# anonymousauthors001/SGS-GNN

Hardware: AMD Instinct MI355X
Metric: sampled edges/sec + training steps/sec, Reddit hybrid 20% sparsity (higher is better)
Workload: dtype f32

## Files before the change

### sgs-gnn_amd/csrc/gemm_tn.hip

```cpp
#include "sgs_common.h"

namespace sgs {
namespace {

using f32x16 = __attribute__((ext_vector_type(16))) float;
constexpr int kUnroll = 8;

__global__ void __launch_bounds__(64) gemm_tn_tile(const float* __restrict__ A, const float* __restrict__ B, int64_t K, int M, int N,
                                                  int ksplit, float* __restrict__ slab) {
    const int lane = threadIdx.x, kh = lane >> 5, l31 = lane & 31;
    const int ti = blockIdx.x, tj = blockIdx.y, s = blockIdx.z;
    const int i = ti * 32 + l31, j = tj * 32 + l31;
    const bool iok = i < M, jok = j < N;
    const int64_t per = ((K + ksplit - 1) / ksplit + 1) & ~int64_t(1);
    const int64_t k0 = s * per, k1 = (k0 + per < K) ? k0 + per : K;
    f32x16 acc;
#pragma unroll
    for (int r = 0; r < 16; ++r) acc[r] = 0.f;
    int64_t k = k0;
    for (; k + 2 * kUnroll <= k1; k += 2 * kUnroll) {
        float a[kUnroll], b[kUnroll];
#pragma unroll
        for (int u = 0; u < kUnroll; ++u) {
            const int64_t kk = k + 2 * u + kh;
// ... 376 lines not shown
                Bp[w][0][m] = p1; Bp[w][1][m] = p2; Bp[w][2][m] = p3;
            }
        if constexpr (MASK) {
#pragma unroll
            for (int t = 0; t < 4; ++t) {
                u32x4 A1;
#pragma unroll
                for (int m = 0; m < 4; ++m)
                    A1[m] = ((r.aw[2 * m] >> t) & 1u) * 0x3F80u + ((r.aw[2 * m + 1] >> t) & 1u) * 0x3F800000u;
                const bf16x8 a1 = __builtin_bit_cast(bf16x8, A1);
#pragma unroll
                for (int w = 0; w < 2; ++w) {
                    if constexpr (ONE) {
                        acc[t][w] = __builtin_amdgcn_mfma_f32_32x32x16_bf16(a1, __builtin_bit_cast(bf16x8, Bp[w][0]), acc[t][w], 0, 0, 0);
                        continue;
                    }
                    const bf16x8 b1 = __builtin_bit_cast(bf16x8, Bp[w][0]), b2 = __builtin_bit_cast(bf16x8, Bp[w][1]), b3 = __builtin_bit_cast(bf16x8, Bp[w][2]);
                    acc[t][w] = __builtin_amdgcn_mfma_f32_32x32x16_bf16(a1, b3, acc[t][w], 0, 0, 0);
                    acc[t][w] = __builtin_amdgcn_mfma_f32_32x32x16_bf16(a1, b2, acc[t][w], 0, 0, 0);
                    acc[t][w] = __builtin_amdgcn_mfma_f32_32x32x16_bf16(a1, b1, acc[t][w], 0, 0, 0);
                }
            }
            return;
        }
#pragma unroll
        for (int t = 0; t < 4; ++t) {
            u32x4 Ap[3];
#pragma unroll
            for (int m = 0; m < 4; ++m) {
                const float4 lo = r.a[2 * m], hi = r.a[2 * m + 1];
                const float e0 = t == 0 ? lo.x : t == 1 ? lo.y : t == 2 ? lo.z : lo.w;
                const float e1 = t == 0 ? hi.x : t == 1 ? hi.y : t == 2 ? hi.z : hi.w;
                uint32_t p1, p2, p3;
                split3(e0, e1, p1, p2, p3);
                Ap[0][m] = p1; Ap[1][m] = p2; Ap[2][m] = p3;
            }
            const bf16x8 a1 = __builtin_bit_cast(bf16x8, Ap[0]), a2 = __builtin_bit_cast(bf16x8, Ap[1]), a3 = __builtin_bit_cast(bf16x8, Ap[2]);
#pragma unroll
            for (int w = 0; w < 2; ++w) {
                const bf16x8 b1 = __builtin_bit_cast(bf16x8, Bp[w][0]), b2 = __builtin_bit_cast(bf16x8, Bp[w][1]), b3 = __builtin_bit_cast(bf16x8, Bp[w][2]);
                acc[t][w] = __builtin_amdgcn_mfma_f32_32x32x16_bf16(a3, b1, acc[t][w], 0, 0, 0);
                acc[t][w] = __builtin_amdgcn_mfma_f32_32x32x16_bf16(a2, b2, acc[t][w], 0, 0, 0);
                acc[t][w] = __builtin_amdgcn_mfma_f32_32x32x16_bf16(a1, b3, acc[t][w], 0, 0, 0);
                acc[t][w] = __builtin_amdgcn_mfma_f32_32x32x16_bf16(a2, b1, acc[t][w], 0, 0, 0);
                acc[t][w] = __builtin_amdgcn_mfma_f32_32x32x16_bf16(a1, b2, acc[t][w], 0, 0, 0);
                acc[t][w] = __builtin_amdgcn_mfma_f32_32x32x16_bf16(a1, b1, acc[t][w], 0, 0, 0);
            }
        }
    };
    Raw r0, r1;
    if constexpr (GATHER) {
        if (lim > 0) {
            Raw r2;
            Idx ix;
            load_idx(k0, ix);
            load_rows(k0, r0, ix);
            load_idx(k0 + 16, ix);
            load_rows(k0 + 16, r1, ix);
            load_idx(k0 + 32, ix);
#pragma unroll 1
            for (int64_t k = k0; k < k1; k += 48) {
                load_rows(k + 32, r2, ix);
                load_idx(k + 48, ix);
                mma(r0);
                load_rows(k + 48, r0, ix);
                load_idx(k + 64, ix);
                mma(r1);
                load_rows(k + 64, r1, ix);
                load_idx(k + 80, ix);
                mma(r2);
            }
        }
    } else if constexpr (!MASK) {
        load(k0, r0);
    } else {
        if (lim > 0) load(k0, r0);
    }
    if constexpr (MASK && !GATHER) {
        if (lim > 0) {
        Raw r2;
        load(k0 + 16, r1);
#pragma unroll 1
        for (int64_t k = k0; k < k1; k += 48) {
            load(k + 32, r2);
            mma(r0);
            load(k + 48, r0);
            mma(r1);
            load(k + 64, r1);
            mma(r2);
        }
        }
    } else if constexpr (!MASK) {
#pragma unroll 1
        for (int64_t k = k0; k < k1; k += 32) {
            load(k + 16, r1);
            mma(r0);
            load(k + 32, r0);
            mma(r1);
        }
    }
    if (want_cs) {
#pragma unroll
        for (int t = 0; t < 4; ++t) cs[t] += __shfl_xor(cs[t], 32, 64);
    }
    if (want_dz) {
        dzs += __shfl_xor(dzs, 32, 64);
        if (lane == 0) dzpart[s] = dzs;
    }
    if (NW > 1) {
        float* csl = red_lds + (NW / 2) * 128 * 64;
#pragma unroll
        for (int half = NW / 2; half >= 1; half >>= 1) {
            if (wave >= half && wave < 2 * half) {
                float* dstp = red_lds + static_cast<size_t>(wave - half) * 128 * 64;
#pragma unroll
                for (int t = 0; t < 4; ++t)
#pragma unroll
                    for (int u = 0; u < 2; ++u)
#pragma unroll
                        for (int r = 0; r < 16; ++r) dstp[((t * 2 + u) * 16 + r) * 64 + lane] = acc[t][u][r];
#pragma unroll
                for (int t = 0; t < 4; ++t) csl[((wave - half) * 4 + t) * 64 + lane] = cs[t];
            }
            __syncthreads();
            if (wave < half) {
                const float* srcp = red_lds + static_cast<size_t>(wave) * 128 * 64;
#pragma unroll
                for (int t = 0; t < 4; ++t)
#pragma unroll
                    for (int u = 0; u < 2; ++u)
#pragma unroll
                        for (int r = 0; r < 16; ++r) acc[t][u][r] += srcp[((t * 2 + u) * 16 + r) * 64 + lane];
#pragma unroll
                for (int t = 0; t < 4; ++t) cs[t] += csl[(wave * 4 + t) * 64 + lane];
            }
            __syncthreads();
        }
        if (wave != 0) return;
    }
    const int slab_id = blockIdx.z;
    if (want_cs && g == 0 && aok) *reinterpret_cast<float4*>(cpart + static_cast<int64_t>(slab_id) * M + ia) = make_float4(cs[0], cs[1], cs[2], cs[3]);
    float* out = slab + static_cast<int64_t>(slab_id) * M * N;
    if (bok) {
#pragma unroll
        for (int t = 0; t < 4; ++t)
#pragma unroll
            for (int r = 0; r < 16; ++r) {
                const int row = m0 + 4 * ((r & 3) + 8 * (r >> 2) + 4 * g) + t;
                if (row < M) *reinterpret_cast<float2*>(out + static_cast<int64_t>(row) * N + jb) = make_float2(acc[t][0][r], acc[t][1][r]);
            }
    }
}

constexpr int maskfeat_stage_words(int MT, int P) { return 2 * P * 64 * 4 + (128 * MT / 32) * 16 + 16; }
constexpr int maskfeat_lds_words(int MT, int P) {
    return 2 * 3 * maskfeat_stage_words(MT, P) > 4 * 2 * 16 * 64 + 4 * MT * 64 + 8 ? 2 * 3 * maskfeat_stage_words(MT, P) : 4 * 2 * 16 * 64 + 4 * MT * 64 + 8;
}
template <int MT, int NG, int P = 3>
__global__ void __launch_bounds__(512) gemm_tn_maskfeat(const uint32_t* __restrict__ Abits, const float* __restrict__ dz,
                                                        const float* __restrict__ codes, const int2* __restrict__ sd, int64_t K, int N,
                                                        float* __restrict__ slab, float* __restrict__ cpart, float* __restrict__ dzpart) {
    constexpr int M = 128 * MT, WPR = M / 32;
    constexpr int kBst = 2 * P * 64 * 4;
    constexpr int kMst = WPR * 16;
    constexpr int kStage = kBst + kMst + 16;
    extern __shared__ uint32_t lds[];
    const int lane = threadIdx.x & 63, g = lane >> 5, l31 = lane & 31;
    const int wave = __builtin_amdgcn_readfirstlane(threadIdx.x >> 6);
    const int kg = wave >> 2, w = wave & 3;
    const int ng = blockIdx.x, n0 = ng * 64, slab_id = blockIdx.y;
    const int64_t per = (((K + gridDim.y - 1) / gridDim.y) + 63) & ~int64_t(63);
    const int64_t kb = static_cast<int64_t>(slab_id) * per + kg * (per >> 1);
    const int64_t ke = (kb + (per >> 1) < K) ? kb + (per >> 1) : K;
    const int nsteps = static_cast<int>(per >> 5);
    const int lim = static_cast<int>(ke - kb);
    uint32_t* st0 = lds + kg * (3 * kStage);
    f32x16 acc[MT][2];
#pragma unroll
    for (int t = 0; t < MT; ++t)
#pragma unroll
        for (int u = 0; u < 2; ++u)
#pragma unroll
            for (int r = 0; r < 16; ++r) acc[t][u][r] = 0.f;
    float cs[MT];
#pragma unroll
    for (int t = 0; t < MT; ++t) cs[t] = 0.f;
    float dzs = 0.f;
    const bool want_cs = cpart != nullptr, want_dz = dzpart != nullptr && ng == 0;
    constexpr int rpg = 8 / NG;
    const int tid_g = threadIdx.x & 255;
    const int srow = (tid_g / WPR) & 15, sword = tid_g % WPR;
    const bool stage_mask = tid_g < 16 * WPR, stage_dz = w == 3 && lane < 16;
    struct S1 { int2 ea, eb; float da, db; uint32_t mw; float dl; };
    struct S2 { float2 as, ad, bs, bd; float da, db; uint32_t mw; float dl; };
    const int64_t kbase = lim > 0 ? kb : 0;
    const int2* sdb = sd + kbase;
    const float* dzb = dz + kbase;
    const uint32_t* abb = Abits + kbase * WPR;
    const int last = lim > 0 ? lim - 1 : 0;
    auto clampr = [&](int rel) { return static_cast<uint32_t>(max(min(rel, last), 0)); };
    const uint32_t coff = static_cast<uint32_t>(n0 + 2 * l31);
    auto load_idx = [&](int step) {
        S1 o;
        const int rel = 16 * step + 8 * g + 2 * w;
        const uint32_t ra = clampr(rel), rb = clampr(rel + 1);
        o.ea = sdb[ra]; o.eb = sdb[rb];
        o.da = dzb[ra]; o.db = dzb[rb];
        o.mw = abb[clampr(16 * step + srow) * WPR + sword];
        o.dl = dzb[clampr(16 * step + (lane & 15))];
        return o;
    };
    auto load_rows = [&](const S1& i) {
        S2 o;
        const uint32_t un = static_cast<uint32_t>(N);
        o.as = *reinterpret_cast<const float2*>(codes + (static_cast<uint32_t>(i.ea.x) * un + coff));
        o.ad = *reinterpret_cast<const float2*>(codes + (static_cast<uint32_t>(i.ea.y) * un + coff));
        o.bs = *reinterpret_cast<const float2*>(codes + (static_cast<uint32_t>(i.eb.x) * un + coff));
        o.bd = *reinterpret_cast<const float2*>(codes + (static_cast<uint32_t>(i.eb.y) * un + coff));
        o.da = i.da; o.db = i.db; o.mw = i.mw; o.dl = i.dl;
        return o;
    };
    auto publish = [&](const S2& r, int step, uint32_t* stg) {
        const int rel = 16 * step + 8 * g + 2 * w;
        const float da = rel < lim ? r.da : 0.f, db = rel + 1 < lim ? r.db : 0.f;
        const float a0 = (r.as.x * r.ad.x) * da, a1 = (r.as.y * r.ad.y) * da;
        const float b0 = (r.bs.x * r.bd.x) * db, b1 = (r.bs.y * r.bd.y) * db;
        if constexpr (P == 1) {
            stg[((0 * P + 0) * 64 + lane) * 4 + w] = pk_bf16(a0, b0);
            stg[((1 * P + 0) * 64 + lane) * 4 + w] = pk_bf16(a1, b1);
        } else {
        uint32_t p1, p2, p3;
        split3(a0, b0, p1, p2, p3);
        stg[((0 * 3 + 0) * 64 + lane) * 4 + w] = p1; stg[((0 * 3 + 1) * 64 + lane) * 4 + w] = p2; stg[((0 * 3 + 2) * 64 + lane) * 4 + w] = p3;
        split3(a1, b1, p1, p2, p3);
        stg[((1 * 3 + 0) * 64 + lane) * 4 + w] = p1; stg[((1 * 3 + 1) * 64 + lane) * 4 + w] = p2; stg[((1 * 3 + 2) * 64 + lane) * 4 + w] = p3;
        }
        if (stage_mask) stg[kBst + sword * 16 + srow] = r.mw;
        if (stage_dz) stg[kBst + kMst + lane] = __float_as_uint(16 * step + lane < lim ? r.dl : 0.f);
        if (want_dz && l31 == 0) dzs += da + db;
    };
    const int wsel = MT * w + ((MT * l31) >> 5), wsh = (MT * l31) & 31;
    struct Ops { bf16x8 bq[2][3]; uint4 m0, m1; uint32_t cw[8 / NG]; float cd[8 / NG]; };
    auto fetch = [&](const uint32_t* stg, Ops& o) {
        o.m0 = *reinterpret_cast<const uint4*>(stg + kBst + wsel * 16 + 8 * g);
        o.m1 = *reinterpret_cast<const uint4*>(stg + kBst + wsel * 16 + 8 * g + 4);
#pragma unroll
        for (int u = 0; u < 2; ++u)
#pragma unroll
            for (int pc = 0; pc < P; ++pc)
                o.bq[u][pc] = __builtin_bit_cast(bf16x8, *reinterpret_cast<const uint4*>(stg + ((u * P + pc) * 64 + lane) * 4));
        if (want_cs) {
#pragma unroll
            for (int jj = 0; jj < rpg; ++jj) {
                const int j = 8 * g + ng * rpg + jj;
                o.cw[jj] = stg[kBst + wsel * 16 + j];
                o.cd[jj] = __uint_as_float(stg[kBst + kMst + j]);
            }
        }
    };
    auto mma = [&](const Ops& o) {
        uint32_t aw[8] = {o.m0.x, o.m0.y, o.m0.z, o.m0.w, o.m1.x, o.m1.y, o.m1.z, o.m1.w};
#pragma unroll
        for (int j = 0; j < 8; ++j) aw[j] >>= wsh;
        uint32_t c[4];
#pragma unroll
        for (int m = 0; m < 4; ++m) c[m] = (aw[2 * m] & ((1u << MT) - 1u)) | ((aw[2 * m + 1] & ((1u << MT) - 1u)) << 16);
#pragma unroll
        for (int t = 0; t < MT; ++t) {
            u32x4 A1;
#pragma unroll
            for (int m = 0; m < 4; ++m) A1[m] = __umul24((c[m] >> t) & 0x00010001u, 0x3F80u);
            const bf16x8 a1 = __builtin_bit_cast(bf16x8, A1);
#pragma unroll
            for (int u = 0; u < 2; ++u) {
                if constexpr (P == 1) {
                    acc[t][u] = __builtin_amdgcn_mfma_f32_32x32x16_bf16(a1, o.bq[u][0], acc[t][u], 0, 0, 0);
                    continue;
                }
                acc[t][u] = __builtin_amdgcn_mfma_f32_32x32x16_bf16(a1, o.bq[u][2], acc[t][u], 0, 0, 0);
                acc[t][u] = __builtin_amdgcn_mfma_f32_32x32x16_bf16(a1, o.bq[u][1], acc[t][u], 0, 0, 0);
                acc[t][u] = __builtin_amdgcn_mfma_f32_32x32x16_bf16(a1, o.bq[u][0], acc[t][u], 0, 0, 0);
            }
        }
        if (want_cs) {
#pragma unroll
            for (int jj = 0; jj < rpg; ++jj) {
                const uint32_t wv = o.cw[jj] >> wsh;
#pragma unroll
                for (int t = 0; t < MT; ++t) cs[t] += (wv >> t) & 1u ? o.cd[jj] : 0.f;
            }
        }
    };
    {
        S1 ia = load_idx(0);
        S2 ra = load_rows(ia);
        S1 ib = load_idx(1);
        S2 rb = load_rows(ib);
        ia = load_idx(2);
        publish(ra, 0, st0);
        int sa = 0, sb = 1;
        if (kg == 1) __syncthreads();
        Ops op;
#pragma unroll 1
        for (int i = 0; i < nsteps; i += 2) {
            ra = load_rows(ia);
            ib = load_idx(i + 3);
            publish(rb, i + 1, st0 + sb * kStage);
            __syncthreads();
            fetch(st0 + sa * kStage, op);
            mma(op);
            __syncthreads();
            sa = sb; sb = sb == 2 ? 0 : sb + 1;
            rb = load_rows(ib);
            ia = load_idx(i + 4);
            publish(ra, i + 2, st0 + sb * kStage);
            __syncthreads();
            fetch(st0 + sa * kStage, op);
            mma(op);
            __syncthreads();
            sa = sb; sb = sb == 2 ? 0 : sb + 1;
        }
        if (kg == 0) __syncthreads();
    }
    if (want_cs) {
#pragma unroll
        for (int t = 0; t < MT; ++t) cs[t] += __shfl_xor(cs[t], 32, 64);
    }
    dzs += __shfl_xor(dzs, 32, 64);
    float* red = reinterpret_cast<float*>(lds);
    constexpr int kRedCs = 4 * 2 * 16 * 64, kRedDz = kRedCs + 4 * MT * 64;
    static_assert(kRedDz + 8 <= maskfeat_lds_words(MT, P) && 2 * 3 * kStage <= maskfeat_lds_words(MT, P), "the K-group sum reuses the stages");
#pragma unroll
    for (int t = 0; t < MT; ++t) {
        __syncthreads();
        if (t == 0 && lane == 0) red[kRedDz + wave] = dzs;
        if (kg == 1) {
#pragma unroll
            for (int u = 0; u < 2; ++u)
#pragma unroll
                for (int r = 0; r < 16; ++r) red[((w * 2 + u) * 16 + r) * 64 + lane] = acc[t][u][r];
            if (t == 0) {
#pragma unroll
                for (int tt = 0; tt < MT; ++tt) red[kRedCs + (w * MT + tt) * 64 + lane] = cs[tt];
            }
        }
        __syncthreads();
        if (kg == 0) {
#pragma unroll
            for (int u = 0; u < 2; ++u)
#pragma unroll
                for (int r = 0; r < 16; ++r) acc[t][u][r] += red[((w * 2 + u) * 16 + r) * 64 + lane];
            if (t == 0) {
#pragma unroll
                for (int tt = 0; tt < MT; ++tt) cs[tt] += red[kRedCs + (w * MT + tt) * 64 + lane];
                if (want_dz && wave == 0 && lane == 0) {
                    float a = 0.f;
                    for (int z = 0; z < 8; ++z) a += red[kRedDz + z];
                    dzpart[slab_id] = a;
                }
            }
        }
    }
    if (kg != 0) return;
    float* out = slab + static_cast<int64_t>(slab_id) * M * N;
#pragma unroll
    for (int t = 0; t < MT; ++t)
#pragma unroll
        for (int r = 0; r < 16; ++r) {
            const int h = 32 * MT * w + MT * ((r & 3) + 8 * (r >> 2) + 4 * g) + t;
            *reinterpret_cast<float2*>(out + static_cast<int64_t>(h) * N + n0 + 2 * l31) = make_float2(acc[t][0][r], acc[t][1][r]);
        }
    if (want_cs && g == 0) {
        float* cp = cpart + (static_cast<int64_t>(slab_id) * NG + ng) * M + 32 * MT * w + MT * l31;
#pragma unroll
        for (int t = 0; t < MT; ++t) cp[t] = cs[t];
    }
}

constexpr int kMaskfeatMaxSlabs = 128;
inline bool use_tall(int64_t K, int64_t M, int64_t N) { return K >= kTallK && M % 4 == 0 && N % 2 == 0; }
inline int pick_ksplit_tall(int64_t K, int64_t M, int64_t N) {
    const int64_t tiles = cdiv(M, 128) * cdiv(N, 64);
    int ks = 1;
    while (ks < 512 && tiles * ks < 1024 && K / (ks * 2) >= 256) ks *= 2;
    return ks;
}

inline int pick_ksplit(int64_t K, int64_t M, int64_t N) {
    if (use_tall(K, M, N)) return pick_ksplit_tall(K, M, N);
    const int64_t tiles = cdiv(M, 32) * cdiv(N, 32);
    int ks = 1;
    while (ks < 64 && tiles * ks < 1024 && K / (ks * 2) >= 64) ks *= 2;
    return ks;
}

inline int wg_waves(int64_t K, int64_t M, int64_t N) {
    if (K <= 0 || M <= 0 || N <= 0 || use_tall(K, M, N)) return 0;
    const int ks = pick_ksplit(K, M, N);
    if (ks == 8 && K >= 512) return 16;
    return (ks == 2 || ks == 4 || ks == 8) ? ks : 0;
}

}
}

using namespace sgs;

extern "C" {

size_t sgs_gemm_tn_workspace_bytes(int64_t K, int64_t M, int64_t N) {
    if (K < 0 || M < 0 || N < 0) return 256;
    const size_t ks = static_cast<size_t>(pick_ksplit(K, M, N));
    return carve_bytes(ks * M * N, 4) + carve_bytes(ks * M, 4) + carve_bytes(kMaskfeatMaxSlabs * 8 * M + kMaskfeatMaxSlabs, 4) + 512;
}

static int gemm_tn_impl(const float* A, const float* B, int64_t K, int64_t M, int64_t N, float* C, float* colsum_A, void* ws,
                        size_t ws_bytes, hipStream_t stream, int64_t ldc = 0, const uint32_t* Abits = nullptr, const float* dz = nullptr,
                        const float* rowscale = nullptr, float scale = 1.f, float* dz_sum = nullptr, float* C_raw = nullptr,
                        float* colsum_raw = nullptr, const int32_t* sd = nullptr, bool one = false);
static int g_tall_bf16x6 = 1;
static int g_gather_shared = 1, g_gather_slabs = 0;
void sgs_gemm_tn_set_gather_variant(int shared, int slabs) { g_gather_shared = shared ? 1 : 0; g_gather_slabs = slabs > 0 ? slabs : 0; }
void sgs_gemm_tn_set_tall_variant(int v) { g_tall_bf16x6 = v < 0 ? 1 : (v ? 1 : 0); }

int sgs_gemm_tn(const float* A, const float* B, int64_t K, int64_t M, int64_t N, float* C, void* ws, size_t ws_bytes,
                sgs_stream_t stream_) {
    return gemm_tn_impl(A, B, K, M, N, C, nullptr, ws, ws_bytes, static_cast<hipStream_t>(stream_));
}

int sgs_gemm_tn_can_colsum(int64_t K, int64_t M, int64_t N) { return use_tall(K, M, N) && pick_ksplit_tall(K, M, N) > 1 ? 1 : 0; }

int sgs_gemm_tn_colsum(const float* A, const float* B, int64_t K, int64_t M, int64_t N, float* C, float* colsum_A, void* ws,
                       size_t ws_bytes, sgs_stream_t stream_) {
    SGS_REQUIRE(colsum_A && sgs_gemm_tn_can_colsum(K, M, N), SGS_EINVAL,
                "sgs_gemm_tn_colsum: shape not served by the tall-K kernel (check sgs_gemm_tn_can_colsum)");
    return gemm_tn_impl(A, B, K, M, N, C, colsum_A, ws, ws_bytes, static_cast<hipStream_t>(stream_));
}

int sgs_gemm_tn_ld(const float* A, const float* B, int64_t K, int64_t M, int64_t N, float* C, int64_t ldc, float* colsum_A, void* ws,
                   size_t ws_bytes, sgs_stream_t stream_) {
    SGS_REQUIRE(ldc >= N, SGS_EINVAL, "sgs_gemm_tn_ld: ldc < N");
    SGS_REQUIRE(!colsum_A || sgs_gemm_tn_can_colsum(K, M, N), SGS_EINVAL, "sgs_gemm_tn_ld: column sums only for the tall-K shapes");
    return gemm_tn_impl(A, B, K, M, N, C, colsum_A, ws, ws_bytes, static_cast<hipStream_t>(stream_), ldc);
}

int sgs_gemm_tn_mask_supported(int64_t K, int64_t M, int64_t N) {
    if (!use_tall(K, M, N) || M % 128 != 0 || N % 64 != 0) return 0;
    const int ks = pick_ksplit_tall(K, M, N);
    return (ks >= 4 && ks % 4 == 0) ? 1 : 0;
}

int sgs_gemm_tn_mask(const uint32_t* Abits, const float* dz, const float* rowscale, float scale, const float* B, int64_t K, int64_t M, int64_t N,
                     float* C, int64_t ldc, float* colsum_A, float* dz_sum, float* C_raw, float* colsum_raw, void* ws, size_t ws_bytes,
                     sgs_stream_t stream_) {
    SGS_REQUIRE(ldc >= N, SGS_EINVAL, "sgs_gemm_tn_mask: ldc < N");
    SGS_REQUIRE(Abits && dz && rowscale, SGS_EINVAL, "sgs_gemm_tn_mask: null pointer");
    SGS_REQUIRE(sgs_gemm_tn_mask_supported(K, M, N), SGS_EINVAL, "sgs_gemm_tn_mask: shape not served (check sgs_gemm_tn_mask_supported)");
    SGS_REQUIRE(!colsum_raw || colsum_A, SGS_EINVAL, "sgs_gemm_tn_mask: colsum_raw needs colsum_A");
    return gemm_tn_impl(nullptr, B, K, M, N, C, colsum_A, ws, ws_bytes, static_cast<hipStream_t>(stream_), ldc, Abits, dz, rowscale, scale, dz_sum,
                        C_raw, colsum_raw);
}

int sgs_gemm_tn_mask_gather(const uint32_t* Abits, const float* dz, const float* rowscale, float scale, const float* codes, int64_t codes_rows,
                            const int32_t* sd, int64_t K, int64_t M, int64_t N, float* C, int64_t ldc, float* colsum_A, float* dz_sum, float* C_raw,
                            float* colsum_raw, void* ws, size_t ws_bytes, sgs_stream_t stream_) {
    SGS_REQUIRE(ldc >= N, SGS_EINVAL, "sgs_gemm_tn_mask_gather: ldc < N");
    SGS_REQUIRE(codes_rows > 0 && codes_rows * N < (int64_t(1) << 32), SGS_EINVAL, "sgs_gemm_tn_mask_gather: the codes table needs 32-bit element offsets");
    SGS_REQUIRE(Abits && dz && rowscale && codes && sd, SGS_EINVAL, "sgs_gemm_tn_mask_gather: null pointer");
    SGS_REQUIRE(sgs_gemm_tn_mask_supported(K, M, N), SGS_EINVAL, "sgs_gemm_tn_mask_gather: shape not served (check sgs_gemm_tn_mask_supported)");
    SGS_REQUIRE(!colsum_raw || colsum_A, SGS_EINVAL, "sgs_gemm_tn_mask_gather: colsum_raw needs colsum_A");
    return gemm_tn_impl(nullptr, codes, K, M, N, C, colsum_A, ws, ws_bytes, static_cast<hipStream_t>(stream_), ldc, Abits, dz, rowscale, scale,
                        dz_sum, C_raw, colsum_raw, sd);
}

int sgs_gemm_tn_mask_bf16(const uint32_t* Abits, const float* dz, const float* rowscale, float scale, const float* B, int64_t K, int64_t M, int64_t N,
                          float* C, int64_t ldc, float* colsum_A, float* dz_sum, float* C_raw, float* colsum_raw, void* ws, size_t ws_bytes,
                          sgs_stream_t stream_) {
    SGS_REQUIRE(ldc >= N, SGS_EINVAL, "sgs_gemm_tn_mask_bf16: ldc < N");
    SGS_REQUIRE(Abits && dz && rowscale, SGS_EINVAL, "sgs_gemm_tn_mask_bf16: null pointer");
    SGS_REQUIRE(sgs_gemm_tn_mask_supported(K, M, N), SGS_EINVAL, "sgs_gemm_tn_mask_bf16: shape not served (check sgs_gemm_tn_mask_supported)");
    SGS_REQUIRE(!colsum_raw || colsum_A, SGS_EINVAL, "sgs_gemm_tn_mask_bf16: colsum_raw needs colsum_A");
    return gemm_tn_impl(nullptr, B, K, M, N, C, colsum_A, ws, ws_bytes, static_cast<hipStream_t>(stream_), ldc, Abits, dz, rowscale, scale, dz_sum,
                        C_raw, colsum_raw, nullptr, true);
}

int sgs_gemm_tn_mask_gather_bf16(const uint32_t* Abits, const float* dz, const float* rowscale, float scale, const float* codes, int64_t codes_rows,
                                 const int32_t* sd, int64_t K, int64_t M, int64_t N, float* C, int64_t ldc, float* colsum_A, float* dz_sum, float* C_raw,
                                 float* colsum_raw, void* ws, size_t ws_bytes, sgs_stream_t stream_) {
    SGS_REQUIRE(ldc >= N, SGS_EINVAL, "sgs_gemm_tn_mask_gather_bf16: ldc < N");
    SGS_REQUIRE(codes_rows > 0 && codes_rows * N < (int64_t(1) << 32), SGS_EINVAL,
                "sgs_gemm_tn_mask_gather_bf16: the codes table needs 32-bit element offsets");
    SGS_REQUIRE(Abits && dz && rowscale && codes && sd, SGS_EINVAL, "sgs_gemm_tn_mask_gather_bf16: null pointer");
    SGS_REQUIRE(sgs_gemm_tn_mask_supported(K, M, N), SGS_EINVAL, "sgs_gemm_tn_mask_gather_bf16: shape not served (check sgs_gemm_tn_mask_supported)");
    SGS_REQUIRE(!colsum_raw || colsum_A, SGS_EINVAL, "sgs_gemm_tn_mask_gather_bf16: colsum_raw needs colsum_A");
    return gemm_tn_impl(nullptr, codes, K, M, N, C, colsum_A, ws, ws_bytes, static_cast<hipStream_t>(stream_), ldc, Abits, dz, rowscale, scale,
                        dz_sum, C_raw, colsum_raw, sd, true);
}

static int gemm_tn_impl(const float* A, const float* B, int64_t K, int64_t M, int64_t N, float* C, float* colsum_A, void* ws,
                        size_t ws_bytes, hipStream_t stream, int64_t ldc, const uint32_t* Abits, const float* dz, const float* rowscale,
                        float scale, float* dz_sum, float* C_raw, float* colsum_raw, const int32_t* sd, bool one) {
    SGS_REQUIRE(K >= 0 && M >= 0 && N >= 0 && M < (1 << 30) && N < (1 << 30), SGS_EINVAL, "sgs_gemm_tn: bad sizes");
    if (M == 0 || N == 0) return SGS_OK;
    SGS_REQUIRE(C && (K == 0 || ((A || Abits) && B)), SGS_EINVAL, "sgs_gemm_tn: null pointer");
    SGS_REQUIRE(ws && ws_bytes >= sgs_gemm_tn_workspace_bytes(K, M, N), SGS_EWORKSPACE, "sgs_gemm_tn: workspace too small");
    const int ks = pick_ksplit(K, M, N);
    Carver cv(ws);
    float* slab = cv.take<float>(static_cast<size_t>(ks) * M * N);
    float* cpart = cv.take<float>(static_cast<size_t>(ks) * M);
    const bool strided = ldc > 0 && ldc != N;
    float* dst = (ks == 1 && !strided) ? C : slab;
    int n_slabs = ks;
    if (Abits) {
        constexpr int NW = 4;
        constexpr size_t lds = (NW / 2) * (128 * 64 + 4 * 64) * sizeof(float);
        static bool raised_m = false;
        if (!raised_m) {
            SGS_HIP_OK(hipFuncSetAttribute(reinterpret_cast<const void*>(&gemm_tn_tall_bf16x6<NW, true>), hipFuncAttributeMaxDynamicSharedMemorySize,
                                           static_cast<int>(lds)));
            raised_m = true;
        }
        n_slabs = ks / NW;
        float* dzpart = dz_sum ? cpart + static_cast<size_t>(n_slabs) * M : nullptr;
        const int NGc = static_cast<int>(N / 64);
        if (sd && g_gather_shared && (M == 128 || M == 256) && N % 64 == 0 && (NGc == 1 || NGc == 2 || NGc == 4 || NGc == 8) && K >= 64) {
            int ns = g_gather_slabs > 0 ? g_gather_slabs : 256 / NGc;
            while (ns > 1 && K / ns < 64) ns >>= 1;
            if (ns > kMaskfeatMaxSlabs) ns = kMaskfeatMaxSlabs;
            if (ns > ks) ns = ks;
            float* cpart2 = cv.take<float>(static_cast<size_t>(kMaskfeatMaxSlabs) * 8 * M + kMaskfeatMaxSlabs);
            float* dzp = dz_sum ? cpart2 + static_cast<size_t>(ns) * NGc * M : nullptr;
            const size_t lds_b = static_cast<size_t>(one ? maskfeat_lds_words(M / 128, 1) : 2 * 3 * (2 * 3 * 64 * 4 + (M / 32) * 16 + 16)) * 4;
            const dim3 grid(static_cast<unsigned>(NGc), static_cast<unsigned>(ns));
            float* cpa = (colsum_A || dz_sum) ? cpart2 : static_cast<float*>(nullptr);
            const int2* sd2 = reinterpret_cast<const int2*>(sd);
            const int Ni = static_cast<int>(N);
#define SGS_MASKFEAT(MT_, NG_)                                                                                                                 \
    do {                                                                                                                                       \
        if (one) hipLaunchKernelGGL((gemm_tn_maskfeat<MT_, NG_, 1>), grid, dim3(512), lds_b, stream, Abits, dz, B, sd2, K, Ni, slab, cpa, dzp);  \
        else     hipLaunchKernelGGL((gemm_tn_maskfeat<MT_, NG_>), grid, dim3(512), lds_b, stream, Abits, dz, B, sd2, K, Ni, slab, cpa, dzp);     \
    } while (0)
            if (M == 256) {
                if (NGc == 1) SGS_MASKFEAT(2, 1); else if (NGc == 2) SGS_MASKFEAT(2, 2); else if (NGc == 4) SGS_MASKFEAT(2, 4); else SGS_MASKFEAT(2, 8);
            } else {
                if (NGc == 1) SGS_MASKFEAT(1, 1); else if (NGc == 2) SGS_MASKFEAT(1, 2); else if (NGc == 4) SGS_MASKFEAT(1, 4); else SGS_MASKFEAT(1, 8);
            }
#undef SGS_MASKFEAT
            hipLaunchKernelGGL(gemm_tn_reduce, dim3(cdiv(M * N + M + 1, 256)), dim3(256), 0, stream, slab, M * N, ns, C,
                               static_cast<const float*>(colsum_A ? cpart2 : nullptr), static_cast<int>(M), colsum_A, static_cast<int>(N),
                               ldc > 0 ? ldc : N, rowscale, scale, static_cast<const float*>(dzp), ns, dz_sum, C_raw, colsum_raw, ns * NGc);
            SGS_LAUNCH_OK();
            return SGS_OK;
        }
        if (one) {
            static bool raised_1 = false;
            if (!raised_1) {
                SGS_HIP_OK(hipFuncSetAttribute(reinterpret_cast<const void*>(&gemm_tn_tall_bf16x6<NW, true, false, true>),
                                               hipFuncAttributeMaxDynamicSharedMemorySize, static_cast<int>(lds)));
                SGS_HIP_OK(hipFuncSetAttribute(reinterpret_cast<const void*>(&gemm_tn_tall_bf16x6<NW, true, true, true>),
                                               hipFuncAttributeMaxDynamicSharedMemorySize, static_cast<int>(lds)));
                raised_1 = true;
            }
            if (sd)
                hipLaunchKernelGGL((gemm_tn_tall_bf16x6<NW, true, true, true>), dim3(cdiv(M, 128), cdiv(N, 64), n_slabs), dim3(64 * NW), lds, stream, A, B,
                                   K, static_cast<int>(M), static_cast<int>(N), ks, slab, (colsum_A || dz_sum) ? cpart : static_cast<float*>(nullptr),
                                   Abits, dz, dzpart, sd);
            else
                hipLaunchKernelGGL((gemm_tn_tall_bf16x6<NW, true, false, true>), dim3(cdiv(M, 128), cdiv(N, 64), n_slabs), dim3(64 * NW), lds, stream, A,
                                   B, K, static_cast<int>(M), static_cast<int>(N), ks, slab, (colsum_A || dz_sum) ? cpart : static_cast<float*>(nullptr),
                                   Abits, dz, dzpart);
        } else if (sd) {
            static bool raised_g = false;
            if (!raised_g) {
                SGS_HIP_OK(hipFuncSetAttribute(reinterpret_cast<const void*>(&gemm_tn_tall_bf16x6<NW, true, true>),
                                               hipFuncAttributeMaxDynamicSharedMemorySize, static_cast<int>(lds)));
                raised_g = true;
            }
            hipLaunchKernelGGL((gemm_tn_tall_bf16x6<NW, true, true>), dim3(cdiv(M, 128), cdiv(N, 64), n_slabs), dim3(64 * NW), lds, stream, A, B, K,
                               static_cast<int>(M), static_cast<int>(N), ks, slab, (colsum_A || dz_sum) ? cpart : static_cast<float*>(nullptr), Abits,
                               dz, dzpart, sd);
        } else
        hipLaunchKernelGGL((gemm_tn_tall_bf16x6<NW, true>), dim3(cdiv(M, 128), cdiv(N, 64), n_slabs), dim3(64 * NW), lds, stream, A, B, K,
                           static_cast<int>(M), static_cast<int>(N), ks, slab, (colsum_A || dz_sum) ? cpart : static_cast<float*>(nullptr), Abits, dz,
                           dzpart);
        hipLaunchKernelGGL(gemm_tn_reduce, dim3(cdiv(M * N + M + 1, 256)), dim3(256), 0, stream, slab, M * N, n_slabs, C,
                           static_cast<const float*>(colsum_A ? cpart : nullptr), static_cast<int>(M), colsum_A, static_cast<int>(N),
                           ldc > 0 ? ldc : N, rowscale, scale, static_cast<const float*>(dzpart), ks, dz_sum, C_raw, colsum_raw);
        SGS_LAUNCH_OK();
        return SGS_OK;
    }
    if (use_tall(K, M, N) && g_tall_bf16x6 && ks >= 4 && ks % 4 == 0) {
        constexpr int NW = 4;
        constexpr size_t lds = (NW / 2) * (128 * 64 + 4 * 64) * sizeof(float);
        static bool raised = false;
        if (!raised) {
            SGS_HIP_OK(hipFuncSetAttribute(reinterpret_cast<const void*>(&gemm_tn_tall_bf16x6<NW>), hipFuncAttributeMaxDynamicSharedMemorySize,
                                           static_cast<int>(lds)));
            raised = true;
        }
        n_slabs = ks / NW;
        hipLaunchKernelGGL((gemm_tn_tall_bf16x6<NW>), dim3(cdiv(M, 128), cdiv(N, 64), n_slabs), dim3(64 * NW), lds, stream, A, B, K,
                           static_cast<int>(M), static_cast<int>(N), ks, slab, colsum_A ? cpart : static_cast<float*>(nullptr));
    } else if (use_tall(K, M, N) && g_tall_bf16x6)
        hipLaunchKernelGGL((gemm_tn_tall_bf16x6<1>), dim3(cdiv(M, 128), cdiv(N, 64), ks), dim3(64), 0, stream, A, B, K, static_cast<int>(M),
                           static_cast<int>(N), ks, dst, colsum_A ? cpart : static_cast<float*>(nullptr));
    else if (use_tall(K, M, N))
        hipLaunchKernelGGL(gemm_tn_tall_tile, dim3(cdiv(M, 128), cdiv(N, 64), ks), dim3(64), 0, stream, A, B, K, static_cast<int>(M),
                           static_cast<int>(N), ks, dst, colsum_A ? cpart : static_cast<float*>(nullptr));
    else if (const int nw = wg_waves(K, M, N)) {
        const dim3 grid(cdiv(M, 32), cdiv(N, 32));
        const int64_t ld = ldc > 0 ? ldc : N;
        if (nw == 16)     hipLaunchKernelGGL((gemm_tn_wg<16>), grid, dim3(1024), 0, stream, A, B, K, static_cast<int>(M), static_cast<int>(N), C, ld);
        else if (nw == 8) hipLaunchKernelGGL((gemm_tn_wg<8>), grid, dim3(512), 0, stream, A, B, K, static_cast<int>(M), static_cast<int>(N), C, ld);
        else if (nw == 4) hipLaunchKernelGGL((gemm_tn_wg<4>), grid, dim3(256), 0, stream, A, B, K, static_cast<int>(M), static_cast<int>(N), C, ld);
        else              hipLaunchKernelGGL((gemm_tn_wg<2>), grid, dim3(128), 0, stream, A, B, K, static_cast<int>(M), static_cast<int>(N), C, ld);
        SGS_LAUNCH_OK();
        return SGS_OK;
    } else
        hipLaunchKernelGGL(gemm_tn_tile, dim3(cdiv(M, 32), cdiv(N, 32), ks), dim3(64), 0, stream, A, B, K, static_cast<int>(M),
                           static_cast<int>(N), ks, dst);
    if (ks > 1 || strided)
        hipLaunchKernelGGL(gemm_tn_reduce, dim3(cdiv(M * N + (colsum_A ? M : 0), 256)), dim3(256), 0, stream, slab, M * N, n_slabs, C,
                           static_cast<const float*>(colsum_A ? cpart : nullptr), static_cast<int>(M), colsum_A, static_cast<int>(N), ldc);
    SGS_LAUNCH_OK();
    return SGS_OK;
}

int sgs_gemm_tn_group_supported(int64_t K, int64_t M, int64_t N) { return wg_waves(K, M, N); }

int sgs_gemm_tn_group(const SgsGemmTnProblem* problems, int count, sgs_stream_t stream_) {
    hipStream_t stream = static_cast<hipStream_t>(stream_);
    SGS_REQUIRE(count >= 0 && (count == 0 || problems), SGS_EINVAL, "sgs_gemm_tn_group: bad problem list");
    for (int p = 0; p < count; ++p) {
        const SgsGemmTnProblem& q = problems[p];
        SGS_REQUIRE(q.K >= 0 && q.M >= 0 && q.N >= 0 && q.M < (1 << 30) && q.N < (1 << 30), SGS_EINVAL, "sgs_gemm_tn_group: bad sizes");
        SGS_REQUIRE(q.ldc == 0 || q.ldc >= q.N, SGS_EINVAL, "sgs_gemm_tn_group: ldc < N");
        SGS_REQUIRE(q.M == 0 || q.N == 0 || (q.C && (q.K == 0 || (q.A && q.B))), SGS_EINVAL, "sgs_gemm_tn_group: null pointer");
    }
    for (int nw = 16; nw >= 2; nw >>= 1) {
        GemmTnGroupArgs a;
        a.count = 0;
        int tiles = 0;
        auto flush = [&]() {
            if (a.count == 0) return;
            for (int z = a.count; z < kGroupMax; ++z) a.d[z] = a.d[0];
            const dim3 grid(static_cast<unsigned>(tiles));
            if (nw == 16)     hipLaunchKernelGGL((gemm_tn_wg_group<16>), grid, dim3(1024), 0, stream, a);
            else if (nw == 8) hipLaunchKernelGGL((gemm_tn_wg_group<8>), grid, dim3(512), 0, stream, a);
            else if (nw == 4) hipLaunchKernelGGL((gemm_tn_wg_group<4>), grid, dim3(256), 0, stream, a);
            else              hipLaunchKernelGGL((gemm_tn_wg_group<2>), grid, dim3(128), 0, stream, a);
            a.count = 0;
            tiles = 0;
        };
        for (int p = 0; p < count; ++p) {
            const SgsGemmTnProblem& q = problems[p];
            if (wg_waves(q.K, q.M, q.N) != nw) continue;
            GemmTnDesc& d = a.d[a.count++];
            d.A = q.A; d.B = q.B; d.C = q.C;
            d.K = q.K; d.ldc = q.ldc > 0 ? q.ldc : q.N;
            d.M = static_cast<int>(q.M); d.N = static_cast<int>(q.N);
            d.first_tile = tiles;
            d.tiles_i = static_cast<int>(cdiv(q.M, 32));
            tiles += d.tiles_i * static_cast<int>(cdiv(q.N, 32));
            if (a.count == kGroupMax) flush();
        }
        flush();
    }
    SGS_LAUNCH_OK();
    for (int p = 0; p < count; ++p) {
        const SgsGemmTnProblem& q = problems[p];
        if (wg_waves(q.K, q.M, q.N) != 0) continue;
        const int rc = gemm_tn_impl(q.A, q.B, q.K, q.M, q.N, q.C, nullptr, q.ws, q.ws_bytes, stream, q.ldc);
        if (rc != SGS_OK) return rc;
    }
    return SGS_OK;
}

}
```

Measured before the change: 107.8 million.

## Software-pipeline the maskfeat gather GEMM loop with split index and row loads

Adds a PIPE variant of the masked gather GEMM kernel. Edge-index loads are split from dz and mask loads so they are issued further ahead, codes-row addresses are computed with 24-bit multiplies on byte offsets, and the next stage's LDS fetch and mask-to-bf16 expansion are interleaved with the current MFMAs through sched_group_barrier hints. The aim is to hide gather latency and VALU expansion work behind matrix ops. It costs more registers, and an optional compile-time timestamp probe is added. The new path is used only when index and size bounds make the 24-bit and 32-bit offset arithmetic safe.

Result: no change. 109.4 million (median of 6 runs) (+1.4%).

```diff
diff --git a/sgs-gnn_amd/csrc/gemm_tn.hip b/sgs-gnn_amd/csrc/gemm_tn.hip
--- a/sgs-gnn_amd/csrc/gemm_tn.hip
+++ b/sgs-gnn_amd/csrc/gemm_tn.hip
@@ -552,11 +552,22 @@
     }
 }
 
+#ifndef SGS_PHASE_PROBE
+#define SGS_PHASE_PROBE 0
+#endif
+#if SGS_PHASE_PROBE
+__device__ unsigned long long* d_maskfeat_trace = nullptr;
+#define SGS_MF_STAMP(k) do { if (w == 0) asm volatile("s_memtime %0\n\ts_waitcnt lgkmcnt(0)" : "=s"(pst[k]) :: "memory"); } while (0)
+#define SGS_MF_SUM() do { if (w == 0) { psum[0] += pst[1] - pst[0]; psum[1] += pst[2] - pst[1]; psum[2] += pst[3] - pst[2]; psum[3] += pst[4] - pst[3]; } } while (0)
+#else
+#define SGS_MF_STAMP(k) do { } while (0)
+#define SGS_MF_SUM() do { } while (0)
+#endif
 constexpr int maskfeat_stage_words(int MT, int P) { return 2 * P * 64 * 4 + (128 * MT / 32) * 16 + 16; }
 constexpr int maskfeat_lds_words(int MT, int P) {
     return 2 * 3 * maskfeat_stage_words(MT, P) > 4 * 2 * 16 * 64 + 4 * MT * 64 + 8 ? 2 * 3 * maskfeat_stage_words(MT, P) : 4 * 2 * 16 * 64 + 4 * MT * 64 + 8;
 }
-template <int MT, int NG, int P = 3>
+template <int MT, int NG, int P = 3, bool PIPE = true>
 __global__ void __launch_bounds__(512) gemm_tn_maskfeat(const uint32_t* __restrict__ Abits, const float* __restrict__ dz,
                                                         const float* __restrict__ codes, const int2* __restrict__ sd, int64_t K, int N,
                                                         float* __restrict__ slab, float* __restrict__ cpart, float* __restrict__ dzpart) {
@@ -620,9 +631,37 @@
         o.da = i.da; o.db = i.db; o.mw = i.mw; o.dl = i.dl;
         return o;
     };
-    auto publish = [&](const S2& r, int step, uint32_t* stg) {
+    struct E { int2 ea, eb; };
+    struct D { float da, db; uint32_t mw; float dl; };
+    struct R { float2 as, ad, bs, bd; };
+    auto at = [](const auto* base, uint32_t byte_off) { return *reinterpret_cast<decltype(base)>(reinterpret_cast<const char*>(base) + byte_off); };
+    auto load_e = [&](int step) {
+        E o;
         const int rel = 16 * step + 8 * g + 2 * w;
-        const float da = rel < lim ? r.da : 0.f, db = rel + 1 < lim ? r.db : 0.f;
+        o.ea = at(sdb, clampr(rel) << 3); o.eb = at(sdb, clampr(rel + 1) << 3);
+        return o;
+    };
+    auto load_d = [&](int step) {
+        D o;
+        const int rel = 16 * step + 8 * g + 2 * w;
+        o.da = at(dzb, clampr(rel) << 2); o.db = at(dzb, clampr(rel + 1) << 2);
+        o.mw = at(abb, (clampr(16 * step + srow) * WPR + sword) << 2);
+        o.dl = at(dzb, clampr(16 * step + (lane & 15)) << 2);
+        return o;
+    };
+    const uint32_t n4 = static_cast<uint32_t>(N) << 2, coff4 = coff << 2;
+    const float2* codes2 = reinterpret_cast<const float2*>(codes);
+    auto load_r = [&](const E& i) {
+        R o;
+        o.as = at(codes2, __umul24(static_cast<uint32_t>(i.ea.x), n4) + coff4);
+        o.ad = at(codes2, __umul24(static_cast<uint32_t>(i.ea.y), n4) + coff4);
+        o.bs = at(codes2, __umul24(static_cast<uint32_t>(i.eb.x), n4) + coff4);
+        o.bd = at(codes2, __umul24(static_cast<uint32_t>(i.eb.y), n4) + coff4);
+        return o;
+    };
+    auto publish = [&](const auto& r, const auto& d, int step, uint32_t* stg) {
+        const int rel = 16 * step + 8 * g + 2 * w;
+        const float da = rel < lim ? d.da : 0.f, db = rel + 1 < lim ? d.db : 0.f;
         const float a0 = (r.as.x * r.ad.x) * da, a1 = (r.as.y * r.ad.y) * da;
         const float b0 = (r.bs.x * r.bd.x) * db, b1 = (r.bs.y * r.bd.y) * db;
         if constexpr (P == 1) {
@@ -635,12 +674,12 @@
         split3(a1, b1, p1, p2, p3);
         stg[((1 * 3 + 0) * 64 + lane) * 4 + w] = p1; stg[((1 * 3 + 1) * 64 + lane) * 4 + w] = p2; stg[((1 * 3 + 2) * 64 + lane) * 4 + w] = p3;
         }
-        if (stage_mask) stg[kBst + sword * 16 + srow] = r.mw;
-        if (stage_dz) stg[kBst + kMst + lane] = __float_as_uint(16 * step + lane < lim ? r.dl : 0.f);
+        if (stage_mask) stg[kBst + sword * 16 + srow] = d.mw;
+        if (stage_dz) stg[kBst + kMst + lane] = __float_as_uint(16 * step + lane < lim ? d.dl : 0.f);
         if (want_dz && l31 == 0) dzs += da + db;
     };
     const int wsel = MT * w + ((MT * l31) >> 5), wsh = (MT * l31) & 31;
-    struct Ops { bf16x8 bq[2][3]; uint4 m0, m1; uint32_t cw[8 / NG]; float cd[8 / NG]; };
+    struct Ops { bf16x8 bq[2][3]; uint4 m0, m1; uint32_t cw[8 / NG]; float cd[8 / NG]; u32x4 af[MT]; };
     auto fetch = [&](const uint32_t* stg, Ops& o) {
         o.m0 = *reinterpret_cast<const uint4*>(stg + kBst + wsel * 16 + 8 * g);
         o.m1 = *reinterpret_cast<const uint4*>(stg + kBst + wsel * 16 + 8 * g + 4);
@@ -658,7 +697,7 @@
             }
         }
     };
-    auto mma = [&](const Ops& o) {
+    auto expand = [&](Ops& o) {
         uint32_t aw[8] = {o.m0.x, o.m0.y, o.m0.z, o.m0.w, o.m1.x, o.m1.y, o.m1.z, o.m1.w};
 #pragma unroll
         for (int j = 0; j < 8; ++j) aw[j] >>= wsh;
@@ -666,11 +705,14 @@
 #pragma unroll
         for (int m = 0; m < 4; ++m) c[m] = (aw[2 * m] & ((1u << MT) - 1u)) | ((aw[2 * m + 1] & ((1u << MT) - 1u)) << 16);
 #pragma unroll
+        for (int t = 0; t < MT; ++t)
+#pragma unroll
+            for (int m = 0; m < 4; ++m) o.af[t][m] = __umul24((c[m] >> t) & 0x00010001u, 0x3F80u);
+    };
+    auto mma_pipe = [&](const Ops& o, Ops& nx) {
+#pragma unroll
         for (int t = 0; t < MT; ++t) {
-            u32x4 A1;
-#pragma unroll
-            for (int m = 0; m < 4; ++m) A1[m] = __umul24((c[m] >> t) & 0x00010001u, 0x3F80u);
-            const bf16x8 a1 = __builtin_bit_cast(bf16x8, A1);
+            const bf16x8 a1 = __builtin_bit_cast(bf16x8, o.af[t]);
 #pragma unroll
             for (int u = 0; u < 2; ++u) {
                 if constexpr (P == 1) {
@@ -682,6 +724,18 @@
                 acc[t][u] = __builtin_amdgcn_mfma_f32_32x32x16_bf16(a1, o.bq[u][0], acc[t][u], 0, 0, 0);
             }
         }
+        expand(nx);
+#pragma unroll
+        for (int t = 0; t < MT; ++t)
+#pragma unroll
+            for (int m = 0; m < 4; ++m) asm volatile("" : "+v"(nx.af[t][m]));
+        constexpr int kMf = 2 * MT * P, kLead = kMf >= 8 ? 4 : kMf / 2;
+        __builtin_amdgcn_sched_group_barrier(0x8, kLead, 0);
+#pragma unroll
+        for (int q = kLead; q < kMf; ++q) {
+            __builtin_amdgcn_sched_group_barrier(0x2, 6, 0);
+            __builtin_amdgcn_sched_group_barrier(0x8, 1, 0);
+        }
         if (want_cs) {
 #pragma unroll
             for (int jj = 0; jj < rpg; ++jj) {
@@ -691,13 +745,99 @@
             }
         }
     };
-    {
+    auto mma = [&](const Ops& o) {
+        uint32_t aw[8] = {o.m0.x, o.m0.y, o.m0.z, o.m0.w, o.m1.x, o.m1.y, o.m1.z, o.m1.w};
+#pragma unroll
+        for (int j = 0; j < 8; ++j) aw[j] >>= wsh;
+        uint32_t c[4];
+#pragma unroll
+        for (int m = 0; m < 4; ++m) c[m] = (aw[2 * m] & ((1u << MT) - 1u)) | ((aw[2 * m + 1] & ((1u << MT) - 1u)) << 16);
+#pragma unroll
+        for (int t = 0; t < MT; ++t) {
+            u32x4 A1;
+#pragma unroll
+            for (int m = 0; m < 4; ++m) A1[m] = __umul24((c[m] >> t) & 0x00010001u, 0x3F80u);
+            const bf16x8 a1 = __builtin_bit_cast(bf16x8, A1);
+#pragma unroll
+            for (int u = 0; u < 2; ++u) {
+                if constexpr (P == 1) {
+                    acc[t][u] = __builtin_amdgcn_mfma_f32_32x32x16_bf16(a1, o.bq[u][0], acc[t][u], 0, 0, 0);
+                    continue;
+                }
+                acc[t][u] = __builtin_amdgcn_mfma_f32_32x32x16_bf16(a1, o.bq[u][2], acc[t][u], 0, 0, 0);
+                acc[t][u] = __builtin_amdgcn_mfma_f32_32x32x16_bf16(a1, o.bq[u][1], acc[t][u], 0, 0, 0);
+                acc[t][u] = __builtin_amdgcn_mfma_f32_32x32x16_bf16(a1, o.bq[u][0], acc[t][u], 0, 0, 0);
+            }
+        }
+        if (want_cs) {
+#pragma unroll
+            for (int jj = 0; jj < rpg; ++jj) {
+                const uint32_t wv = o.cw[jj] >> wsh;
+#pragma unroll
+                for (int t = 0; t < MT; ++t) cs[t] += (wv >> t) & 1u ? o.cd[jj] : 0.f;
+            }
+        }
+    };
+#if SGS_PHASE_PROBE
+    unsigned long long pst[5] = {0, 0, 0, 0, 0}, psum[4] = {0, 0, 0, 0};
+#endif
+    if constexpr (PIPE) {
+        E ea = load_e(0), eb = load_e(1);
+        D da = load_d(0), db = load_d(1);
+        R ra = load_r(ea);
+        R rb = load_r(eb);
+        publish(ra, da, 0, st0);
+        ea = load_e(2);
+        da = load_d(2);
+        eb = load_e(3);
+        int sa = 0, sb = 1;
+        Ops oa, ob;
+        __syncthreads();
+        fetch(st0, oa);
+        expand(oa);
+        if (kg == 1) __syncthreads();
+#pragma unroll 1
+        for (int i = 0; i < nsteps; i += 2) {
+            SGS_MF_STAMP(0);
+            ra = load_r(ea);
+            publish(rb, db, i + 1, st0 + sb * kStage);
+            ea = load_e(i + 4);
+            db = load_d(i + 3);
+            SGS_MF_STAMP(1);
+            __syncthreads();
+            SGS_MF_STAMP(2);
+            fetch(st0 + sb * kStage, ob);
+            mma_pipe(oa, ob);
+            SGS_MF_STAMP(3);
+            __syncthreads();
+            SGS_MF_STAMP(4);
+            SGS_MF_SUM();
+            sa = sb; sb = sb == 2 ? 0 : sb + 1;
+            SGS_MF_STAMP(0);
+            rb = load_r(eb);
+            publish(ra, da, i + 2, st0 + sb * kStage);
+            eb = load_e(i + 5);
+            da = load_d(i + 4);
+            SGS_MF_STAMP(1);
+            __syncthreads();
+            SGS_MF_STAMP(2);
+            fetch(st0 + sb * kStage, oa);
+            mma_pipe(ob, oa);
+            SGS_MF_STAMP(3);
+            __syncthreads();
+            SGS_MF_STAMP(4);
+            SGS_MF_SUM();
+            sa = sb; sb = sb == 2 ? 0 : sb + 1;
+        }
+        (void)sa;
+        if (kg == 0) __syncthreads();
+    } else {
         S1 ia = load_idx(0);
         S2 ra = load_rows(ia);
         S1 ib = load_idx(1);
         S2 rb = load_rows(ib);
         ia = load_idx(2);
-        publish(ra, 0, st0);
+        publish(ra, ra, 0, st0);
         int sa = 0, sb = 1;
         if (kg == 1) __syncthreads();
         Ops op;
@@ -705,23 +845,41 @@
         for (int i = 0; i < nsteps; i += 2) {
             ra = load_rows(ia);
             ib = load_idx(i + 3);
-            publish(rb, i + 1, st0 + sb * kStage);
+            SGS_MF_STAMP(0);
+            publish(rb, rb, i + 1, st0 + sb * kStage);
+            SGS_MF_STAMP(1);
             __syncthreads();
+            SGS_MF_STAMP(2);
             fetch(st0 + sa * kStage, op);
             mma(op);
+            SGS_MF_STAMP(3);
             __syncthreads();
+            SGS_MF_STAMP(4);
+            SGS_MF_SUM();
             sa = sb; sb = sb == 2 ? 0 : sb + 1;
             rb = load_rows(ib);
             ia = load_idx(i + 4);
-            publish(ra, i + 2, st0 + sb * kStage);
+            SGS_MF_STAMP(0);
+            publish(ra, ra, i + 2, st0 + sb * kStage);
+            SGS_MF_STAMP(1);
             __syncthreads();
+            SGS_MF_STAMP(2);
             fetch(st0 + sa * kStage, op);
             mma(op);
+            SGS_MF_STAMP(3);
             __syncthreads();
+            SGS_MF_STAMP(4);
+            SGS_MF_SUM();
             sa = sb; sb = sb == 2 ? 0 : sb + 1;
         }
         if (kg == 0) __syncthreads();
     }
+#if SGS_PHASE_PROBE
+    if (d_maskfeat_trace && w == 0 && lane == 0) {
+        unsigned long long* tr = d_maskfeat_trace + ((static_cast<size_t>(blockIdx.y) * gridDim.x + blockIdx.x) * 2 + kg) * 4;
+        for (int k = 0; k < 4; ++k) tr[k] = psum[k];
+    }
+#endif
     if (want_cs) {
 #pragma unroll
         for (int t = 0; t < MT; ++t) cs[t] += __shfl_xor(cs[t], 32, 64);
@@ -817,10 +975,16 @@
 static int gemm_tn_impl(const float* A, const float* B, int64_t K, int64_t M, int64_t N, float* C, float* colsum_A, void* ws,
                         size_t ws_bytes, hipStream_t stream, int64_t ldc = 0, const uint32_t* Abits = nullptr, const float* dz = nullptr,
                         const float* rowscale = nullptr, float scale = 1.f, float* dz_sum = nullptr, float* C_raw = nullptr,
-                        float* colsum_raw = nullptr, const int32_t* sd = nullptr, bool one = false);
+                        float* colsum_raw = nullptr, const int32_t* sd = nullptr, bool one = false, int64_t codes_rows = 0);
 static int g_tall_bf16x6 = 1;
 static int g_gather_shared = 1, g_gather_slabs = 0;
-void sgs_gemm_tn_set_gather_variant(int shared, int slabs) { g_gather_shared = shared ? 1 : 0; g_gather_slabs = slabs > 0 ? slabs : 0; }
+void sgs_gemm_tn_set_gather_variant(int shared, int slabs) { g_gather_shared = shared == 2 ? 2 : (shared ? 1 : 0); g_gather_slabs = slabs > 0 ? slabs : 0; }
+#if SGS_PHASE_PROBE
+int sgs_gemm_tn_maskfeat_probe_trace(unsigned long long* buf) {
+    SGS_HIP_OK(hipMemcpyToSymbol(HIP_SYMBOL(d_maskfeat_trace), &buf, sizeof(buf)));
+    return SGS_OK;
+}
+#endif
 void sgs_gemm_tn_set_tall_variant(int v) { g_tall_bf16x6 = v < 0 ? 1 : (v ? 1 : 0); }
 
 int sgs_gemm_tn(const float* A, const float* B, int64_t K, int64_t M, int64_t N, float* C, void* ws, size_t ws_bytes,
@@ -870,7 +1034,7 @@
     SGS_REQUIRE(sgs_gemm_tn_mask_supported(K, M, N), SGS_EINVAL, "sgs_gemm_tn_mask_gather: shape not served (check sgs_gemm_tn_mask_supported)");
     SGS_REQUIRE(!colsum_raw || colsum_A, SGS_EINVAL, "sgs_gemm_tn_mask_gather: colsum_raw needs colsum_A");
     return gemm_tn_impl(nullptr, codes, K, M, N, C, colsum_A, ws, ws_bytes, static_cast<hipStream_t>(stream_), ldc, Abits, dz, rowscale, scale,
-                        dz_sum, C_raw, colsum_raw, sd);
+                        dz_sum, C_raw, colsum_raw, sd, false, codes_rows);
 }
 
 int sgs_gemm_tn_mask_bf16(const uint32_t* Abits, const float* dz, const float* rowscale, float scale, const float* B, int64_t K, int64_t M, int64_t N,
@@ -894,12 +1058,12 @@
     SGS_REQUIRE(sgs_gemm_tn_mask_supported(K, M, N), SGS_EINVAL, "sgs_gemm_tn_mask_gather_bf16: shape not served (check sgs_gemm_tn_mask_supported)");
     SGS_REQUIRE(!colsum_raw || colsum_A, SGS_EINVAL, "sgs_gemm_tn_mask_gather_bf16: colsum_raw needs colsum_A");
     return gemm_tn_impl(nullptr, codes, K, M, N, C, colsum_A, ws, ws_bytes, static_cast<hipStream_t>(stream_), ldc, Abits, dz, rowscale, scale,
-                        dz_sum, C_raw, colsum_raw, sd, true);
+                        dz_sum, C_raw, colsum_raw, sd, true, codes_rows);
 }
 
 static int gemm_tn_impl(const float* A, const float* B, int64_t K, int64_t M, int64_t N, float* C, float* colsum_A, void* ws,
                         size_t ws_bytes, hipStream_t stream, int64_t ldc, const uint32_t* Abits, const float* dz, const float* rowscale,
-                        float scale, float* dz_sum, float* C_raw, float* colsum_raw, const int32_t* sd, bool one) {
+                        float scale, float* dz_sum, float* C_raw, float* colsum_raw, const int32_t* sd, bool one, int64_t codes_rows) {
     SGS_REQUIRE(K >= 0 && M >= 0 && N >= 0 && M < (1 << 30) && N < (1 << 30), SGS_EINVAL, "sgs_gemm_tn: bad sizes");
     if (M == 0 || N == 0) return SGS_OK;
     SGS_REQUIRE(C && (K == 0 || ((A || Abits) && B)), SGS_EINVAL, "sgs_gemm_tn: null pointer");
@@ -935,10 +1099,14 @@
             float* cpa = (colsum_A || dz_sum) ? cpart2 : static_cast<float*>(nullptr);
             const int2* sd2 = reinterpret_cast<const int2*>(sd);
             const int Ni = static_cast<int>(N);
+            const bool pipe = g_gather_shared != 2 && K < (int64_t(1) << 26) && codes_rows < (int64_t(1) << 24) && N < (1 << 22) &&
+                              codes_rows * N < (int64_t(1) << 30);
 #define SGS_MASKFEAT(MT_, NG_)                                                                                                                 \
     do {                                                                                                                                       \
-        if (one) hipLaunchKernelGGL((gemm_tn_maskfeat<MT_, NG_, 1>), grid, dim3(512), lds_b, stream, Abits, dz, B, sd2, K, Ni, slab, cpa, dzp);  \
-        else     hipLaunchKernelGGL((gemm_tn_maskfeat<MT_, NG_>), grid, dim3(512), lds_b, stream, Abits, dz, B, sd2, K, Ni, slab, cpa, dzp);     \
+        if (one) { if (pipe) hipLaunchKernelGGL((gemm_tn_maskfeat<MT_, NG_, 1, true>), grid, dim3(512), lds_b, stream, Abits, dz, B, sd2, K, Ni, slab, cpa, dzp);     \
+                   else      hipLaunchKernelGGL((gemm_tn_maskfeat<MT_, NG_, 1, false>), grid, dim3(512), lds_b, stream, Abits, dz, B, sd2, K, Ni, slab, cpa, dzp); }  \
+        else     { if (pipe) hipLaunchKernelGGL((gemm_tn_maskfeat<MT_, NG_, 3, true>), grid, dim3(512), lds_b, stream, Abits, dz, B, sd2, K, Ni, slab, cpa, dzp);     \
+                   else      hipLaunchKernelGGL((gemm_tn_maskfeat<MT_, NG_, 3, false>), grid, dim3(512), lds_b, stream, Abits, dz, B, sd2, K, Ni, slab, cpa, dzp); }  \
     } while (0)
             if (M == 256) {
                 if (NGc == 1) SGS_MASKFEAT(2, 1); else if (NGc == 2) SGS_MASKFEAT(2, 2); else if (NGc == 4) SGS_MASKFEAT(2, 4); else SGS_MASKFEAT(2, 8);
```
